# larskaislaniemi/PyLamp

Hardware: AMD Instinct MI355X
Metric: stokes_heat_mic_cell_updates_per_s (higher is better)
Workload: dtype f64

## Files before the change

pylamp_amd/csrc/pl_solver.hip:

```cpp
#include "pl_internal.h"
#include <chrono>
#include <cmath>
#include <functional>
#include <limits>

#define TB(tab, k) (tab)[(k) + PL_TOFF]

void pl_launch_heat_rhs(pl_ctx* ctx, const PlHeatOp& op, const double* Told, const double* H, double* rhs);

template <typename T>
struct PlVvOpT {
    PlGeom g;
    const T* etas; const T* etan;
    const T *rdz, *rDz, *rdx, *rDx;
    int slave_x;
    int slave_z0, slave_zL;
    T s0, sL;
    const T* szz; const T* szx;
};
typedef PlVvOpT<double> PlVvOp;
typedef PlVvOpT<float> PlVvOpF;

enum { VV_ZERO = 0, VV_INT = 1, VV_SLAVE = 2 };

// ... 1295 lines not shown
    float *etas_f = nullptr, *etan_f = nullptr, *tab_f = nullptr;
    float* vf[3] = {nullptr, nullptr, nullptr};
    float *ff = nullptr, *rf = nullptr;
};
template <typename T> struct LevelT;
template <> struct LevelT<double> {
    static const PlVvOp& op(const MgLevel* L) { return L->op; }
    static double** v(MgLevel* L) { return L->v; }
    static double* f(MgLevel* L) { return L->f; }
    static double* r(MgLevel* L) { return L->r; }
};
template <> struct LevelT<float> {
    static const PlVvOpF& op(const MgLevel* L) { return L->opf; }
    static float** v(MgLevel* L) { return L->vf; }
    static float* f(MgLevel* L) { return L->ff; }
    static float* r(MgLevel* L) { return L->rf; }
};

struct PlSolver {
    std::vector<MgLevel*> levels;
    int bc_key[4] = {-1, -1, -1, -1};
    int repl_start = -1;
    long long repl_max_nodes = 300000;
    double *r = nullptr, *rt = nullptr, *p = nullptr, *v = nullptr, *s = nullptr, *t = nullptr, *y = nullptr,
           *z = nullptr, *b = nullptr, *x = nullptr, *xb = nullptr, *dx = nullptr, *r0 = nullptr, *xh = nullptr,
           *bu = nullptr;
    double* scal = nullptr;
    double* hpart = nullptr;
    double* epi = nullptr;
    long long epi_blocks = 0;
    int nu_pre = 2, nu_post = 2, coarse_sweeps = 12;
    int nu0_pre = -1, nu0_post = -1;
    bool aniso_auto = true, ratio_knob = false;
    int power_its_warm = 1;
    bool nu_auto = true;
    bool use_tail = true;
    bool any_line = false;
    long long tail_knob = 0;
    long long tail_max_nodes = 33 * 33;
    int min_cells = 4;
    bool f32_enable = false; long long f32_min_nodes = 200000;
    double etol = 3e-8;
    double kappa = 1.0, sigma = 1.0;
    bool defl_enable = true;
    bool defl_persistent = false;
    bool defl_valid = false, defl_active = false;
    double *wdefl = nullptr, *udefl = nullptr;
    double defl_yAw = 0.0, defl_wvel2 = 0.0;
    double* Awdefl = nullptr;
    bool defl_lazy = false;
    double schur_scale = 1.0;
    double ref_cached = 0.0, ref_kc = 0.0; int ref_age = 0;
    long long fused_max_nodes = 1100000;
    long long tile32_min_nodes = 1000000;
    bool fused = true;
    bool fuse_first = true;
    bool l0_mixed = true;
    bool l0_mixed_now = true;
    bool deep = true;
    int tail_nu_pre = -1, tail_nu_post = -1;
    double cheb_ratio = 6.0, lmax_safety = 1.1;
    double* h[11] = {nullptr};
    double* hc3 = nullptr;
    double* hc[9] = {nullptr}; double* hc_part = nullptr; int hc_nb = 0, hc_last_its = 0;
    int napply = 0, nprec = 0;
    long long heat_fused_launches = 0;
    long long tail_lds_launches = 0, tail_global_launches = 0;
};

static PlSolver* solver_of(pl_ctx* ctx) {
    if (!ctx->krylov) {
        PlSolver* S = new PlSolver();
        if (const char* e = getenv("PYLAMP_MG_NU")) { int a = 0, b = 0; if (sscanf(e, "%d,%d", &a, &b) == 2 && a >= 0 && b >= 0 && a + b > 0) { S->nu_pre = a; S->nu_post = b; S->nu_auto = false; } }
        if (const char* e = getenv("PYLAMP_MG_NU0")) { int a = 0, b = 0; if (sscanf(e, "%d,%d", &a, &b) == 2 && a >= 1 && b >= 1) { S->nu0_pre = a; S->nu0_post = b; S->nu_auto = false; } }
        if (const char* e = getenv("PYLAMP_MG_POWER")) { int a = atoi(e); if (a >= 1) S->power_its_warm = a; }
        if (const char* e = getenv("PYLAMP_MG_COARSE")) { int a = atoi(e); if (a > 0) S->coarse_sweeps = a; }
        if (const char* e = getenv("PYLAMP_MG_TAIL")) S->use_tail = atoi(e) != 0;
        if (const char* e = getenv("PYLAMP_MG_REPL_NODES")) { long long v = atoll(e); if (v >= 25) S->repl_max_nodes = v; }
        if (const char* e = getenv("PYLAMP_MG_TAIL_NODES")) { long long v = atoll(e); if (v >= 25 && v <= PL_TAIL_MAX_NODES) S->tail_knob = v; }
        if (const char* e = getenv("PYLAMP_MG_DEEP")) S->deep = atoi(e) != 0;
        if (const char* e = getenv("PYLAMP_DEFLATE")) S->defl_enable = atoi(e) != 0;
        if (const char* e = getenv("PYLAMP_STOKES_ETOL")) { const double v = atof(e); if (v >= 0.0) S->etol = v; }
        if (const char* e = getenv("PYLAMP_MG_FP32")) S->f32_enable = atoi(e) != 0;
        if (const char* e = getenv("PYLAMP_MG_FP32_NODES")) { long long v = atoll(e); if (v >= 1) S->f32_min_nodes = v; }
        if (const char* e = getenv("PYLAMP_L0_MIXED")) S->l0_mixed = atoi(e) != 0;
        if (const char* e = getenv("PYLAMP_MG_FUSED")) S->fused = atoi(e) != 0;
        if (const char* e = getenv("PYLAMP_MG_TS32")) { long long v = atoll(e); if (v > 0) S->tile32_min_nodes = v; }
        if (const char* e = getenv("PYLAMP_MG_FUSED_MAX")) { long long v = atoll(e); if (v > 0) S->fused_max_nodes = v; }
        if (const char* e = getenv("PYLAMP_SCHUR_SCALE")) { double v = atof(e); if (v > 0.0) S->schur_scale = v; }
        if (const char* e = getenv("PYLAMP_MG_TAIL_NU")) { int a = 0, b = 0; if (sscanf(e, "%d,%d", &a, &b) == 2 && a + b > 0) { S->tail_nu_pre = a; S->tail_nu_post = b; } }
        if (const char* e = getenv("PYLAMP_MG_RATIO")) { double v = atof(e); if (v > 1.5) { S->cheb_ratio = v; S->ratio_knob = true; } }
        if (const char* e = getenv("PYLAMP_MG_ANISO")) S->aniso_auto = atoi(e) != 0;
        if (const char* e = getenv("PYLAMP_MG_SAFETY")) { double v = atof(e); if (v >= 1.0) S->lmax_safety = v; }
        ctx->krylov = S;
    }
    return (PlSolver*)ctx->krylov;
}

static void free_levels(PlSolver* S) {
    for (MgLevel* L : S->levels) {
        if (L->own_visc) { (void)hipFree(L->etas); (void)hipFree(L->etan); }
        if (L->own_rho && L->rho) (void)hipFree(L->rho);
        for (double* q : {L->szz, L->szx, L->eig}) if (q) (void)hipFree(q);
        for (double* q : {L->v[0], L->v[1], L->v[2], L->f, L->r}) if (q) (void)hipFree(q);
        for (float* q : {L->etas_f, L->etan_f, L->tab_f, L->vf[0], L->vf[1], L->vf[2], L->ff, L->rf}) if (q) (void)hipFree(q);
        pl_geom_free(L->gh);
        delete L;
// ... 656 lines not shown
            hipLaunchKernelGGL(k_vv_residual<T>, pl_grid_rows(V.op.g), dim3(64, 4), 0, ctx->stream, V.op, (const T*)(buf[0] - V.sh), f - V.sh,
                               r - V.sh, pl_row_iters(V.op.g));
    } else {
        smooth<T>(ctx, L, buf, f, npre, S->cheb_ratio, nullptr, 1.0, true, false, -1, first_done_anchor);
        if (L->dist) (void)pl_halo(ctx, g, buf[0], 2, g.plane);
        if (g_vv_vec)
            hipLaunchKernelGGL((k_vv_sweep2<1, T, T>), pl_grid_rows2(g), dim3(64, 4), 0, ctx->stream, LevelT<T>::op(L), (const T*)buf[0], (const T*)nullptr, f,
                               r, T(0), T(0), T(1));
        else
            hipLaunchKernelGGL(k_vv_residual<T>, pl_grid_rows(g), dim3(64, 4), 0, ctx->stream, LevelT<T>::op(L), (const T*)buf[0], f, r, pl_row_iters(g));
        if (L->dist) (void)pl_halo(ctx, g, r, 2, g.plane, 2);
    }
    if constexpr (std::is_same<T, float>::value) {
        if (C->f32) coarse_correction<float, float>(ctx, S, l, L, C, buf, deep, npost);
        else coarse_correction<float, double>(ctx, S, l, L, C, buf, deep, npost);
    } else {
        coarse_correction<double, double>(ctx, S, l, L, C, buf, deep, npost);
    }
    std::swap(buf[0], buf[2]);
    if (deep) *wrote_final = smooth<T>(ctx, L, buf, f, npost, S->cheb_ratio, final_out, final_scale, false, true, npost - 1);
    else *wrote_final = smooth<T>(ctx, L, buf, f, npost, S->cheb_ratio, final_out, final_scale, false, L->dist);
    *out = buf[0];
}

#define MGT_TS 16
#ifndef MGT_NT
#define MGT_NT 1024
#endif
struct MgTileArgs {
    PlVvOp op;
    PlVvOp opc;
    const double* f; double* fout;
    double* v;
    double* fc;
    const double* ec;
    double* out; double oscale; long long out_plane;
    double c1[4], c2[4];
    PlStokesOp sop; const double* rs; double* z;
    int tiles_x;
};

struct MgtTab { const double* es; const double* en; const double* rdz; const double* rDz; const double* rdx; const double* rDx; };

__device__ inline int mgt_cls_z(const PlVvOp& op, int i, int j, int& db, double& s) {
    db = 0; s = 1.0;
    if (i <= 0 || i >= op.g.nz - 1 || j < 0 || j >= op.g.nx - 1) return VV_ZERO;
    if (op.slave_x) {
        if (j == 0) { db = 1; return VV_SLAVE; }
        if (j == op.g.nx - 2) { db = -1; return VV_SLAVE; }
    }
    return VV_INT;
}
__device__ inline int mgt_cls_x(const PlVvOp& op, int i, int j, int& da, double& s) {
    da = 0; s = 1.0;
    if (j <= 0 || j >= op.g.nx - 1 || i < 0 || i >= op.g.nz - 1) return VV_ZERO;
    if (i == 0 && op.slave_z0) { da = 1; s = op.s0; return VV_SLAVE; }
    if (i == op.g.nz - 2 && op.slave_zL) { da = -1; s = op.sL; return VV_SLAVE; }
    return VV_INT;
}
__device__ inline void mgt_load_table(double* dst, const double* tab, int first_global, int count, int n) {
    for (int k = threadIdx.x; k < count; k += blockDim.x) {
        const int gk = first_global + k;
        dst[k] = (gk >= -PL_TOFF && gk < n + PL_TOFF) ? TB(tab, gk) : 0.0;
    }
}

struct MgtC { double c0, c1, c2, c3, x0, x1, rdg, s, f; int cm, d; bool on, interior; };
template <bool ZC>
__device__ inline MgtC mgt_classify(const PlVvOp& op, int CR, int NR, int ci0, int cj0, int a, int b) {
    MgtC k; k.c0 = k.c1 = k.c2 = k.c3 = k.x0 = k.x1 = k.rdg = k.f = 0.0; k.s = 1.0; k.cm = a * CR + b; k.d = 0; k.on = false; k.interior = false;
    if (a < 1 || a > NR - 2 || b < 1 || b > CR - 2) return k;
    int d; double s;
    const int cls = ZC ? mgt_cls_z(op, ci0 + a, cj0 + b, d, s) : mgt_cls_x(op, ci0 + a, cj0 + b, d, s);
    const int am = ZC ? a : a + d, bm = ZC ? b + d : b;
    if (cls == VV_ZERO || am < 1 || am > NR - 2 || bm < 1 || bm > CR - 2) return k;
    k.s = s; k.cm = am * CR + bm; k.d = d; k.on = true; k.interior = cls == VV_INT;
    return k;
}
template <bool ZC>
__device__ inline void mgt_coefficients(MgtC& k, const MgtTab& t, int CR) {
    if (!k.on) return;
    const int c = k.cm, am = c / CR, bm = c - am * CR;
    if (ZC) {
        const double rdz_i = t.rdz[am + 1], rdz_m = t.rdz[am], rDz_i = t.rDz[am + 1];
        const double rdx_j = t.rdx[bm + 1], rDx_j = t.rDx[bm + 1], rDx_p = t.rDx[bm + 2];
        const double esC = t.es[c], esE = t.es[c + 1];
        k.c0 = 4.0 * t.en[c] * rdz_i * rDz_i; k.c1 = 4.0 * t.en[c - CR] * rdz_m * rDz_i;
        k.c2 = 2.0 * esE * rDx_p * rdx_j; k.c3 = 2.0 * esC * rDx_j * rdx_j;
        k.x0 = 2.0 * esE * rDz_i * rdx_j; k.x1 = 2.0 * esC * rDz_i * rdx_j;
    } else {
        const double rdx_j = t.rdx[bm + 1], rdx_m = t.rdx[bm], rDx_j = t.rDx[bm + 1];
        const double rdz_i = t.rdz[am + 1], rDz_i = t.rDz[am + 1], rDz_p = t.rDz[am + 2];
        const double esC = t.es[c], esN = t.es[c + CR];
        k.c0 = 4.0 * t.en[c] * rdx_j * rDx_j; k.c1 = 4.0 * t.en[c - 1] * rdx_m * rDx_j;
        k.c2 = 2.0 * esN * rDz_p * rdz_i; k.c3 = 2.0 * esC * rDz_i * rdz_i;
        k.x0 = 2.0 * esN * rDx_j * rdz_i; k.x1 = 2.0 * esC * rDx_j * rdz_i;
    }
    k.rdg = pl_rcp(k.c0 + k.c1 + k.c2 + k.c3);
}
__device__ inline double mgt_dg(const MgtC& k) { return k.c0 + k.c1 + k.c2 + k.c3; }
__device__ inline double mgt_av_z(const MgtC& k, int CR, const double* vz, const double* vx, double& v0) {
    const int c = k.cm; v0 = vz[c];
    return k.c0 * (vz[c + CR] - v0) - k.c1 * (v0 - vz[c - CR]) + k.c2 * (vz[c + 1] - v0) - k.c3 * (v0 - vz[c - 1]) +
           k.x0 * (vx[c + 1] - vx[c - CR + 1]) - k.x1 * (vx[c] - vx[c - CR]);
}
__device__ inline double mgt_av_x(const MgtC& k, int CR, const double* vz, const double* vx, double& v0) {
    const int c = k.cm; v0 = vx[c];
    return k.c0 * (vx[c + 1] - v0) - k.c1 * (v0 - vx[c - 1]) + k.c2 * (vx[c + CR] - v0) - k.c3 * (v0 - vx[c - CR]) +
           k.x0 * (vz[c + CR] - vz[c + CR - 1]) - k.x1 * (vz[c] - vz[c - 1]);
}
__device__ inline void mgt_cheb(const MgtC& kz, const MgtC& kx, int CR, const double* vz, const double* vx, double& pvz, double& pvx,
                                double c1, double c2, double& oz, double& ox) {
    oz = 0.0; ox = 0.0;
    if (kz.on) {
        double v0; const double Av = mgt_av_z(kz, CR, vz, vx, v0);
        const double mom = (c1 != 0.0) ? c1 * (v0 - pvz) : 0.0;
        oz = kz.s * (v0 + mom + (c2 * (Av - kz.f)) * kz.rdg);
        pvz = v0;
    }
    if (kx.on) {
        double v0; const double Av = mgt_av_x(kx, CR, vz, vx, v0);
        const double mom = (c1 != 0.0) ? c1 * (v0 - pvx) : 0.0;
        ox = kx.s * (v0 + mom + (c2 * (Av - kx.f)) * kx.rdg);
        pvx = v0;
    }
}
__device__ inline bool mgt_owns(int ra, int rb, int HC, int TS, int i, int j, const PlGeom& g) {
    return ra >= HC && (ra < HC + TS || (ra == HC + TS && i == g.nz - 1)) && rb >= HC && (rb < HC + TS || (rb == HC + TS && j == g.nx - 1));
}
__host__ __device__ constexpr int mgt_npt(int nn) { return (nn + 1023) / 1024; }
__host__ __device__ constexpr int mgt_nt(int nn) { return ((nn + mgt_npt(nn) - 1) / mgt_npt(nn) + 63) / 64 * 64; }
__host__ __device__ constexpr int mgt_pre_nn(int NS, int TS) { return (TS + 2 * (NS + 2)) * (TS + 2 * (NS + 2)); }
__host__ __device__ constexpr int mgt_post_nn(int NS, int TS) { return (TS + 2 * (NS + 1)) * (TS + 2 * (NS + 1)); }

template <int NS, bool L0, int TS, int EXT = 0>
__global__ __launch_bounds__(mgt_nt(mgt_pre_nn(NS + EXT, TS))) void k_mg_pre(MgTileArgs a) {
    constexpr int H = NS + 1 + EXT, HC = H + 1, CR = TS + 2 * HC, NN = CR * CR, NPT = mgt_npt(NN), NT = mgt_nt(NN);
    __shared__ double V[2][2][NN];
    __shared__ double ZP[L0 ? NN : 1];
    __shared__ double TAB[4][CR + 4];
    double* const ES = V[1][0]; double* const EN = V[1][1];
    const PlGeom& g = a.op.g;
    const int tid = threadIdx.x;
    const int ty = blockIdx.x / a.tiles_x, tx = blockIdx.x % a.tiles_x;
    const int ti0 = g.gi0 + ty * TS, tj0 = g.gj0 + tx * TS;
    const int ci0 = ti0 - HC, cj0 = tj0 - HC;
    MgtTab t; t.es = ES; t.en = EN; t.rdz = TAB[0]; t.rDz = TAB[1]; t.rdx = TAB[2]; t.rDx = TAB[3];
    mgt_load_table(TAB[0], a.op.rdz, ci0 - 1, CR + 3, g.nz); mgt_load_table(TAB[1], a.op.rDz, ci0 - 1, CR + 3, g.nz);
    mgt_load_table(TAB[2], a.op.rdx, cj0 - 1, CR + 3, g.nx); mgt_load_table(TAB[3], a.op.rDx, cj0 - 1, CR + 3, g.nx);
    const long long P = g.plane;
    MgtC kz[NPT], kx[NPT];
    int depth[NPT];
#pragma unroll
    for (int q = 0; q < NPT; q++) {
        const int idx = tid + q * NT;
        const bool have = idx < NN;
        const int ra = have ? idx / CR : 0, rb = have ? idx % CR : 0, i = ci0 + ra, j = cj0 + rb;
        depth[q] = have ? min(min(ra, CR - 1 - ra), min(rb, CR - 1 - rb)) : -1;
        kz[q] = mgt_classify<true>(a.op, CR, CR, ci0, cj0, ra, rb);
        kx[q] = mgt_classify<false>(a.op, CR, CR, ci0, cj0, ra, rb);
        const bool inmem = i - g.gi0 >= -PL_RING && i - g.gi0 < g.lnz + PL_RING && j - g.gj0 >= -PL_RING && j - g.gj0 < g.lnx + PL_RING;
        const long long c = pl_idx(g, i - g.gi0, j - g.gj0);
        const double* const fsrc = L0 ? a.rs : a.f;
        if (kz[q].on) kz[q].f = fsrc[c + kz[q].d];
        if (kx[q].on) kx[q].f = fsrc[c + (long long)kx[q].d * g.pitch + P];
        if (have) {
            ES[idx] = inmem ? a.op.etas[c] : 0.0; EN[idx] = inmem ? a.op.etan[c] : 0.0;
            if (L0) {
                const bool indom = i >= 0 && i < g.nz && j >= 0 && j < g.nx;
                ZP[idx] = indom ? prec_p_value(a.sop, a.rs + 2 * P, i, j, c) : 0.0;
            }
        }
    }
    __syncthreads();
#pragma unroll
    for (int q = 0; q < NPT; q++) {
        mgt_coefficients<true>(kz[q], t, CR); mgt_coefficients<false>(kx[q], t, CR);
        if (L0) {
            const int idx = tid + q * NT;
            const int ra = depth[q] >= 0 ? idx / CR : 0, rb = depth[q] >= 0 ? idx % CR : 0, i = ci0 + ra, j = cj0 + rb;
            if (kz[q].on) kz[q].f = kz[q].f * mgt_dg(kz[q]) + 2.0 * a.sop.Kc * TAB[1][ra + 1] * (ZP[kz[q].cm] - ZP[kz[q].cm - CR]);
            if (kx[q].on) kx[q].f = kx[q].f * mgt_dg(kx[q]) + 2.0 * a.sop.Kc * TAB[3][rb + 1] * (ZP[kx[q].cm] - ZP[kx[q].cm - 1]);
            if (depth[q] >= 0 && mgt_owns(ra, rb, HC, TS, i, j, g) && i < g.nz && j < g.nx && i - g.gi0 < g.lnz && j - g.gj0 < g.lnx) {
                const long long c = pl_idx(g, i - g.gi0, j - g.gj0);
                a.fout[c] = kz[q].interior ? kz[q].f : 0.0; a.fout[c + P] = kx[q].interior ? kx[q].f : 0.0; a.z[c + 2 * P] = ZP[idx];
            }
        }
    }
    int cur = 0;
#pragma unroll
    for (int q = 0; q < NPT; q++) {
        const int idx = tid + q * NT;
        if (depth[q] >= HC - H) {
            V[0][0][idx] = kz[q].on ? (-kz[q].s * a.c2[0] * kz[q].f) * kz[q].rdg : 0.0;
            V[0][1][idx] = kx[q].on ? (-kx[q].s * a.c2[0] * kx[q].f) * kx[q].rdg : 0.0;
        }
    }
    __syncthreads();
    double pvz[NPT], pvx[NPT];
#pragma unroll
    for (int q = 0; q < NPT; q++) { pvz[q] = 0.0; pvx[q] = 0.0; }
#pragma unroll
    for (int k = 1; k < NS; k++) {
        const int h = H - k;
#pragma unroll
        for (int q = 0; q < NPT; q++) {
            const int idx = tid + q * NT;
            if (depth[q] >= HC - h) {
                double oz, ox;
                mgt_cheb(kz[q], kx[q], CR, V[cur][0], V[cur][1], pvz[q], pvx[q], a.c1[k], a.c2[k], oz, ox);
                V[cur ^ 1][0][idx] = oz; V[cur ^ 1][1][idx] = ox;
            }
        }
        __syncthreads();
        cur ^= 1;
    }
    const int nxt = cur ^ 1;
#pragma unroll
    for (int q = 0; q < NPT; q++) {
        const int idx = tid + q * NT;
        if (depth[q] >= HC - 1) {
            double v0, rz = 0.0, rx = 0.0;
            if (kz[q].interior) rz = kz[q].f - mgt_av_z(kz[q], CR, V[cur][0], V[cur][1], v0);
            if (kx[q].interior) rx = kx[q].f - mgt_av_x(kx[q], CR, V[cur][0], V[cur][1], v0);
            V[nxt][0][idx] = rz; V[nxt][1][idx] = rx;
        }
        if (depth[q] >= HC - (EXT ? NS : 1)) {
            const int ra = idx / CR, rb = idx % CR, i = ci0 + ra, j = cj0 + rb, li = i - g.gi0, lj = j - g.gj0;
            const bool owned = li >= 0 && li < g.lnz && lj >= 0 && lj < g.lnx;
            const bool ring = EXT && !owned && li >= -NS && li < g.lnz + NS && lj >= -NS && lj < g.lnx + NS;
            if (i >= 0 && i < g.nz && j >= 0 && j < g.nx && ((owned && mgt_owns(ra, rb, HC, TS, i, j, g)) || ring)) {
                const long long c = pl_idx(g, li, lj);
                a.v[c] = V[cur][0][idx]; a.v[c + P] = V[cur][1][idx];
            }
        }
    }
    __syncthreads();
    const PlGeom& gc = a.opc.g;
    for (int idx = tid; idx < (TS / 2 + 1) * (TS / 2 + 1); idx += NT) {
        const int u_ = idx / (TS / 2 + 1), w_ = idx % (TS / 2 + 1);
        const int I = (ti0 >> 1) + u_, J = (tj0 >> 1) + w_;
        if ((u_ == TS / 2 && I != gc.nz - 1) || (w_ == TS / 2 && J != gc.nx - 1)) continue;
        if (I >= gc.nz || J >= gc.nx || 2 * I - g.gi0 >= g.lnz || 2 * J - g.gj0 >= g.lnx) continue;
        const int b0 = (2 * I - ci0) * CR + (2 * J - cj0);
        int d; double s;
        double oz = 0.0, ox = 0.0;
        if (vv_cls_z(a.opc, I, J, d, s) == VV_INT) {
            const double wz[3] = {0.25, 0.5, 0.25}, wx[4] = {0.125, 0.375, 0.375, 0.125};
#pragma unroll
            for (int u = 0; u < 3; u++)
#pragma unroll
                for (int w = 0; w < 4; w++) oz += wz[u] * wx[w] * V[nxt][0][b0 + (u - 1) * CR + (w - 1)];
        }
        if (vv_cls_x(a.opc, I, J, d, s) == VV_INT) {
            const double wz[4] = {0.125, 0.375, 0.375, 0.125}, wx[3] = {0.25, 0.5, 0.25};
#pragma unroll
            for (int u = 0; u < 4; u++)
#pragma unroll
                for (int w = 0; w < 3; w++) ox += wz[u] * wx[w] * V[nxt][1][b0 + (u - 1) * CR + (w - 1)];
        }
        const long long cc = pl_idx(gc, I - gc.gi0, J - gc.gj0);
        a.fc[cc] = oz; a.fc[cc + gc.plane] = ox;
    }
}

template <int NS, int TS>
__global__ __launch_bounds__(mgt_nt(mgt_post_nn(NS, TS))) void k_mg_post(MgTileArgs a) {
    constexpr int H = NS, HC = H + 1, CR = TS + 2 * HC, NN = CR * CR, ECR = TS / 2 + H + 6, ENN = ECR * ECR, NPT = mgt_npt(NN), NT = mgt_nt(NN);
    __shared__ double V[2][2][NN];
    __shared__ double EC[2][ENN];
    __shared__ double TAB[4][CR + 4];
    double* const ES = V[0][0]; double* const EN = V[0][1];
    const PlGeom& g = a.op.g; const PlGeom& gc = a.opc.g;
    const int tid = threadIdx.x;
    const int ty = blockIdx.x / a.tiles_x, tx = blockIdx.x % a.tiles_x;
    const int ti0 = g.gi0 + ty * TS, tj0 = g.gj0 + tx * TS;
    const int ci0 = ti0 - HC, cj0 = tj0 - HC;
    MgtTab t; t.es = ES; t.en = EN; t.rdz = TAB[0]; t.rDz = TAB[1]; t.rdx = TAB[2]; t.rDx = TAB[3];
    mgt_load_table(TAB[0], a.op.rdz, ci0 - 1, CR + 3, g.nz); mgt_load_table(TAB[1], a.op.rDz, ci0 - 1, CR + 3, g.nz);
    mgt_load_table(TAB[2], a.op.rdx, cj0 - 1, CR + 3, g.nx); mgt_load_table(TAB[3], a.op.rDx, cj0 - 1, CR + 3, g.nx);
    const long long P = g.plane;
    const int eI0 = ((ti0 - H) >> 1) - 2, eJ0 = ((tj0 - H) >> 1) - 2;
    MgtC kz[NPT], kx[NPT];
    int depth[NPT];
#pragma unroll
    for (int q = 0; q < NPT; q++) {
        const int idx = tid + q * NT;
        const bool have = idx < NN;
        const int ra = have ? idx / CR : 0, rb = have ? idx % CR : 0, i = ci0 + ra, j = cj0 + rb;
        depth[q] = have ? min(min(ra, CR - 1 - ra), min(rb, CR - 1 - rb)) : -1;
        kz[q] = mgt_classify<true>(a.op, CR, CR, ci0, cj0, ra, rb);
        kx[q] = mgt_classify<false>(a.op, CR, CR, ci0, cj0, ra, rb);
        const bool inmem = i - g.gi0 >= -PL_RING && i - g.gi0 < g.lnz + PL_RING && j - g.gj0 >= -PL_RING && j - g.gj0 < g.lnx + PL_RING;
        const long long c = pl_idx(g, i - g.gi0, j - g.gj0);
        if (kz[q].on) kz[q].f = a.f[c + kz[q].d];
        if (kx[q].on) kx[q].f = a.f[c + (long long)kx[q].d * g.pitch + P];
        if (have) {
            ES[idx] = inmem ? a.op.etas[c] : 0.0; EN[idx] = inmem ? a.op.etan[c] : 0.0;
            V[1][0][idx] = inmem ? a.v[c] : 0.0; V[1][1][idx] = inmem ? a.v[c + P] : 0.0;
        }
    }
    for (int idx = tid; idx < ENN; idx += NT) {
        const int I = eI0 + idx / ECR, J = eJ0 + idx % ECR;
        const bool inmem = I - gc.gi0 >= -PL_RING && I - gc.gi0 < gc.lnz + PL_RING && J - gc.gj0 >= -PL_RING && J - gc.gj0 < gc.lnx + PL_RING;
        const long long cc = pl_idx(gc, I - gc.gi0, J - gc.gj0);
        EC[0][idx] = inmem ? a.ec[cc] : 0.0; EC[1][idx] = inmem ? a.ec[cc + gc.plane] : 0.0;
    }
    __syncthreads();
#pragma unroll
    for (int q = 0; q < NPT; q++) { mgt_coefficients<true>(kz[q], t, CR); mgt_coefficients<false>(kx[q], t, CR); }
    __syncthreads();
    auto ecz = [&](int I, int J) { return EC[0][(I - eI0) * ECR + (J - eJ0)]; };
    auto ecx = [&](int I, int J) { return EC[1][(I - eI0) * ECR + (J - eJ0)]; };
#pragma unroll
    for (int q = 0; q < NPT; q++) {
        const int idx = tid + q * NT;
        if (depth[q] >= HC - H) {
            const int ra = idx / CR, rb = idx % CR, i = ci0 + ra, j = cj0 + rb;
            int d; double s;
            double oz = 0.0, ox = 0.0;
            if (mgt_cls_z(a.op, i, j, d, s) != VV_ZERO) {
                const int jm = j + d;
                const int I0 = i >> 1, I1 = (i + 1) >> 1;
                int Jn = jm >> 1, Jo = (jm & 1) ? Jn + 1 : Jn - 1;
                Jn = min(max(Jn, 0), gc.nx - 2); Jo = min(max(Jo, 0), gc.nx - 2);
                const double pa = 0.5 * (ecz(I0, Jn) + ecz(I1, Jn)), pb = 0.5 * (ecz(I0, Jo) + ecz(I1, Jo));
                oz = s * (V[1][0][idx + d] + (0.75 * pa + 0.25 * pb));
            }
            if (mgt_cls_x(a.op, i, j, d, s) != VV_ZERO) {
                const int im = i + d;
                const int J0 = j >> 1, J1 = (j + 1) >> 1;
                int In = im >> 1, Io = (im & 1) ? In + 1 : In - 1;
                In = min(max(In, 0), gc.nz - 2); Io = min(max(Io, 0), gc.nz - 2);
                const double pa = 0.5 * (ecx(In, J0) + ecx(In, J1)), pb = 0.5 * (ecx(Io, J0) + ecx(Io, J1));
                ox = s * (V[1][1][idx + d * CR] + (0.75 * pa + 0.25 * pb));
            }
            V[0][0][idx] = oz; V[0][1][idx] = ox;
        }
    }
    __syncthreads();
    int cur = 0;
    double pvz[NPT], pvx[NPT];
#pragma unroll
    for (int q = 0; q < NPT; q++) { pvz[q] = 0.0; pvx[q] = 0.0; }
#pragma unroll
    for (int k = 0; k < NS; k++) {
        const int h = H - 1 - k;
#pragma unroll
        for (int q = 0; q < NPT; q++) {
            const int idx = tid + q * NT;
            if (depth[q] >= HC - h) {
                double oz, ox;
                mgt_cheb(kz[q], kx[q], CR, V[cur][0], V[cur][1], pvz[q], pvx[q], k == 0 ? 0.0 : a.c1[k], a.c2[k], oz, ox);
                if (k == NS - 1) {
                    const int ra = idx / CR, rb = idx % CR, i = ci0 + ra, j = cj0 + rb;
                    if (i < g.nz && j < g.nx && i - g.gi0 < g.lnz && j - g.gj0 < g.lnx) {
                        const long long c = pl_idx(g, i - g.gi0, j - g.gj0); a.out[c] = oz * a.oscale; a.out[c + a.out_plane] = ox * a.oscale;
                    }
                } else { V[cur ^ 1][0][idx] = oz; V[cur ^ 1][1][idx] = ox; }
            }
        }
        if (k < NS - 1) { __syncthreads(); cur ^= 1; }
    }
#pragma unroll
    for (int q = 0; q < NPT; q++) {
        const int idx = tid + q * NT;
        if (depth[q] == HC - 1) {
            const int ra = idx / CR, rb = idx % CR, i = ci0 + ra, j = cj0 + rb;
            if (mgt_owns(ra, rb, HC, TS, i, j, g) && i - g.gi0 < g.lnz && j - g.gj0 < g.lnx) {
                const long long c = pl_idx(g, i - g.gi0, j - g.gj0); a.out[c] = 0.0; a.out[c + a.out_plane] = 0.0;
            }
        }
    }
}

#define MGT_TAIL_POOL 18600
#define MGT_TAIL_CHEB 256
#define MGT_TAIL_LDS 11520
struct TailLvl { int base, NR, CR, N; };
#define TL_V(D, buf, c) (pool + (D).base + (2 * (buf) + (c)) * (D).N)
#define TL_ES(D) (pool + (D).base + 4 * (D).N)
#define TL_EN(D) (pool + (D).base + 5 * (D).N)
#define TL_TAB(D, k) (pool + (D).base + 6 * (D).N + ((k) < 2 ? (k) * ((D).NR + 3) : 2 * ((D).NR + 3) + ((k) - 2) * ((D).CR + 3)))
__host__ __device__ inline TailLvl mgt_tail_lvl(const PlGeom& g, int base) {
    TailLvl D; D.base = base; D.NR = g.nz + 2; D.CR = g.nx + 2; D.N = D.NR * D.CR;
    return D;
}
__host__ __device__ inline int mgt_tail_lvl_size(const TailLvl& D) { return 6 * D.N + 2 * (D.NR + 3) + 2 * (D.CR + 3); }
// ... 262 lines not shown
        need += 10LL * (g.nz + 2) * (g.nx + 2) + 2LL * (g.nz + 5) + 2LL * (g.nx + 5);
        lds += mgt_tail_lvl_size(mgt_tail_lvl(g, 0)); table_entries += 2LL * (g.nz + 5) + 2LL * (g.nx + 5);
        if (q > l) { coarse_threads = (coarse_threads + 63) / 64 * 64 + (long long)(g.nz - 1) * (g.nx - 1); coarse_nodes += (long long)g.nz * g.nx; }
    }
    const PlGeom& g0 = S->levels[l]->gh.d;
    return need <= MGT_TAIL_POOL && lds <= MGT_TAIL_LDS && (long long)(g0.nz - 1) * (g0.nx - 1) <= MGT_NT && (long long)g0.nz * g0.nx <= 2 * MGT_NT &&
           coarse_threads <= MGT_NT && coarse_nodes <= MGT_NT && table_entries <= MGT_NT;
}

static void cheb_coeffs(double lmax, double ratio, int n, double* c1, double* c2) {
    const double lmin = lmax / ratio, theta = 0.5 * (lmax + lmin), delta = 0.5 * (lmax - lmin), sigma = theta / delta;
    double rho_old = 1.0 / sigma;
    for (int k = 0; k < n; k++) {
        if (k == 0) { c1[k] = 0.0; c2[k] = 1.0 / theta; }
        else { const double rho = 1.0 / (2.0 * sigma - rho_old); c1[k] = rho * rho_old; c2[k] = 2.0 * rho / delta; rho_old = rho; }
    }
}
static bool mg_fused_level_ok(pl_ctx* ctx, const PlSolver* S, size_t l) {
    if (!S->fused || l + 1 >= S->levels.size() || S->any_line) return false;
    const MgLevel* L = S->levels[l];
    if (L->f32 || L->op.szz) return false;
    const PlGeom& g = L->gh.d;
    int npre_, npost_;
    level_nu(S, l, npre_, npost_);
    if (L->dist) {
        const bool dist_fused = !(getenv("PYLAMP_MG_FUSED_DIST") && atoi(getenv("PYLAMP_MG_FUSED_DIST")) == 0);
        const MgLevel* C = S->levels[l + 1];
        if (!dist_fused || l == 0 || npre_ + 2 > std::min(g.lnz, g.lnx) || npre_ + 3 > PL_RING) return false;
        if (C->dist && std::min(C->gh.d.lnz, C->gh.d.lnx) < 4) return false;
        if ((g.gi0 & 1) || (g.gj0 & 1)) return false;
    } else if (S->levels[l + 1]->dist) return false;
    if ((long long)g.lnz * g.lnx > S->fused_max_nodes) return false;
    if (S->use_tail && l > 0 && (long long)g.nz * g.nx <= S->tail_max_nodes && S->levels.size() - l <= PL_TAIL_MAX_LEVELS) return false;
    int npre, npost;
    level_nu(S, l, npre, npost);
    return npre >= 1 && npre <= 3 && npost >= 1 && npost <= 3;
}
static void vcycle_fused_level(pl_ctx* ctx, PlSolver* S, size_t l, const double* f, double** out, double* final_out, double final_scale,
                               const PlStokesOp* sop, const double* rs, double* z) {
    MgLevel* L = S->levels[l];
    MgLevel* C = S->levels[l + 1];
    const PlGeom& g = L->gh.d;
    int npre, npost;
    level_nu(S, l, npre, npost);
    MgTileArgs a{};
    a.op = L->op; a.opc = C->op;
    a.f = rs ? (const double*)L->f : f; a.fout = L->f; a.v = L->v[0]; a.fc = C->f;
    const int TS = (long long)g.lnz * g.lnx >= S->tile32_min_nodes ? 32 : MGT_TS;
    const int own_z = g.lnz - (g.gi0 + g.lnz == g.nz ? 1 : 0), own_x = g.lnx - (g.gj0 + g.lnx == g.nx ? 1 : 0);
    a.tiles_x = (own_x + TS - 1) / TS;
    const dim3 grid((unsigned)(a.tiles_x * ((own_z + TS - 1) / TS)));
    cheb_coeffs(L->lmax, S->cheb_ratio, npre, a.c1, a.c2);
    if (rs) { a.sop = *sop; a.rs = rs; a.z = z; }
#define MGT_PRE(NS, L0) do { if (TS == 32) hipLaunchKernelGGL((k_mg_pre<NS, L0, 32>), grid, dim3(mgt_nt(mgt_pre_nn(NS, 32))), 0, ctx->stream, a); \
                             else hipLaunchKernelGGL((k_mg_pre<NS, L0, MGT_TS>), grid, dim3(mgt_nt(mgt_pre_nn(NS, MGT_TS))), 0, ctx->stream, a); } while (0)
#define MGT_PRE_X(NS) do { if (TS == 32) hipLaunchKernelGGL((k_mg_pre<NS, false, 32, 1>), grid, dim3(mgt_nt(mgt_pre_nn(NS + 1, 32))), 0, ctx->stream, a); \
                           else hipLaunchKernelGGL((k_mg_pre<NS, false, MGT_TS, 1>), grid, dim3(mgt_nt(mgt_pre_nn(NS + 1, MGT_TS))), 0, ctx->stream, a); } while (0)
    if (L->dist) {
        (void)pl_halo(ctx, g, (double*)a.f, 2, g.plane, npre + 2);
        if (npre == 1) MGT_PRE_X(1); else if (npre == 2) MGT_PRE_X(2); else MGT_PRE_X(3);
        if (!C->dist) (void)pl_gather_blocks(ctx, C->gh.d, C->f, 2, C->gh.d.plane);
    }
    else if (rs) { if (npre == 1) MGT_PRE(1, true); else if (npre == 2) MGT_PRE(2, true); else MGT_PRE(3, true); }
    else { if (npre == 1) MGT_PRE(1, false); else if (npre == 2) MGT_PRE(2, false); else MGT_PRE(3, false); }
#undef MGT_PRE
#undef MGT_PRE_X
    double* ec = nullptr;
    bool wf = false;
    vcycle<double>(ctx, S, l + 1, C->f, &ec, &wf, nullptr, 1.0, 0, nullptr);
    if (L->dist && C->dist) (void)pl_halo(ctx, C->gh.d, ec, 2, C->gh.d.plane, 4);
    a.ec = ec; a.out = final_out ? final_out : L->v[2]; a.oscale = final_out ? final_scale : 1.0; a.out_plane = g.plane;
    cheb_coeffs(L->lmax, S->cheb_ratio, npost, a.c1, a.c2);
#define MGT_POST(NS) do { if (TS == 32) hipLaunchKernelGGL((k_mg_post<NS, 32>), grid, dim3(mgt_nt(mgt_post_nn(NS, 32))), 0, ctx->stream, a); \
                          else hipLaunchKernelGGL((k_mg_post<NS, MGT_TS>), grid, dim3(mgt_nt(mgt_post_nn(NS, MGT_TS))), 0, ctx->stream, a); } while (0)
    if (npost == 1) MGT_POST(1); else if (npost == 2) MGT_POST(2); else MGT_POST(3);
#undef MGT_POST
    *out = final_out ? nullptr : L->v[2];
}

template <typename T>
__global__ __launch_bounds__(256) void k_copy_vel(PlGeom g, const T* __restrict__ e, double* __restrict__ z, double oscale) {
    PL_NODE_PROLOGUE(g)
    (void)i; (void)j;
    z[c] = (double)e[c] * oscale; z[c + g.plane] = (double)e[c + g.plane] * oscale;
}

__global__ __launch_bounds__(256) void k_vv_close_frame(PlVvOp op, double* __restrict__ z) {
    const PlGeom& g = op.g;
    const int t = blockIdx.x * 256 + threadIdx.x;
    int i, j;
    if (t < 3 * g.lnx) { const int q = t / g.lnx; i = q == 0 ? 0 : g.nz - 3 + q; j = g.gj0 + t % g.lnx; }
    else if (t < 3 * g.lnx + 3 * g.lnz) { const int u = t - 3 * g.lnx, q = u / g.lnz; j = q == 0 ? 0 : g.nx - 3 + q; i = g.gi0 + u % g.lnz; }
    else return;
    const int li = i - g.gi0, lj = j - g.gj0;
    if (li < 0 || li >= g.lnz || lj < 0 || lj >= g.lnx) return;
    const long long c = pl_idx(g, li, lj), P = g.plane;
    int moff; double s;
    int cls = vv_cls_z(op, i, j, moff, s);
    if (cls == VV_ZERO) z[c] = 0.0; else if (cls == VV_SLAVE) z[c] = s * z[c + moff];
    cls = vv_cls_x(op, i, j, moff, s);
    if (cls == VV_ZERO) z[c + P] = 0.0; else if (cls == VV_SLAVE) z[c + P] = s * z[c + moff + P];
}

template <typename T>
static int stokes_precond_t(pl_ctx* ctx, PlSolver* S, const double* rs, double* z) {
    PlStokesOp op = ctx->sop;
    MgLevel* L0 = S->levels[0];
    MgLevel* L = L0;
    const PlGeom& g = ctx->sop.g;
    const bool f32 = std::is_same<T, float>::value;
    const double kappa = f32 ? S->kappa : 1.0, fscale = f32 ? S->kappa / S->sigma : 1.0, oscale = f32 ? 1.0 / S->kappa : 1.0;
    int e_last = 0, f_depth = 0;
    const bool deep = level_deep_plan(S, L0, 0, e_last, f_depth);
    ExtViewT<T> V = ext_view<T>(ctx, L0, deep ? f_depth : 0);
    if (L0->dist) {
        if (deep) PL_TRY(pl_halo(ctx, g, (double*)rs, 3, g.plane, f_depth + 1));
        else PL_TRY(pl_halo(ctx, g, (double*)rs + 2 * g.plane, 1, g.plane));
    }
    op.g = V.op.g; op.etas -= V.sh; op.etan -= V.sh; if (op.rho) op.rho -= V.sh;
// ... 1481 lines not shown
```

Measured before the change: 199.4 million.

## Batch all global loads into registers before shared-memory stores in multigrid tile kernels

Restructures the prologue of the fused multigrid pre/post smoothing kernels so every global load (viscosities, coordinate tables, RHS, velocities, coarse correction) is issued up front into registers, and only then written to shared memory. The goal is more memory-level parallelism and less serialized load latency per block. Table loads now use one wave per table, with wave-uniform branching and clamped addresses replacing predicated loads. It also lowers the node threshold for switching to 32-wide tiles, which costs more registers per thread and may reduce occupancy.

```diff
diff --git a/pylamp_amd/csrc/pl_solver.hip b/pylamp_amd/csrc/pl_solver.hip
--- a/pylamp_amd/csrc/pl_solver.hip
+++ b/pylamp_amd/csrc/pl_solver.hip
@@ -1371,7 +1371,7 @@
     double schur_scale = 1.0;
     double ref_cached = 0.0, ref_kc = 0.0; int ref_age = 0;
     long long fused_max_nodes = 1100000;
-    long long tile32_min_nodes = 1000000;
+    long long tile32_min_nodes = 250000;
     bool fused = true;
     bool fuse_first = true;
     bool l0_mixed = true;
@@ -2134,19 +2134,14 @@
     return VV_INT;
 }
 __device__ inline int mgt_cls_x(const PlVvOp& op, int i, int j, int& da, double& s) {
+    const double s0 = op.s0, sL = op.sL;
     da = 0; s = 1.0;
     if (j <= 0 || j >= op.g.nx - 1 || i < 0 || i >= op.g.nz - 1) return VV_ZERO;
-    if (i == 0 && op.slave_z0) { da = 1; s = op.s0; return VV_SLAVE; }
-    if (i == op.g.nz - 2 && op.slave_zL) { da = -1; s = op.sL; return VV_SLAVE; }
-    return VV_INT;
-}
-__device__ inline void mgt_load_table(double* dst, const double* tab, int first_global, int count, int n) {
-    for (int k = threadIdx.x; k < count; k += blockDim.x) {
-        const int gk = first_global + k;
-        dst[k] = (gk >= -PL_TOFF && gk < n + PL_TOFF) ? TB(tab, gk) : 0.0;
-    }
-}
-
+    if (i == 0 && op.slave_z0) da = 1;
+    else if (i == op.g.nz - 2 && op.slave_zL) da = -1;
+    s = da > 0 ? s0 : (da < 0 ? sL : 1.0);
+    return da ? VV_SLAVE : VV_INT;
+}
 struct MgtC { double c0, c1, c2, c3, x0, x1, rdg, s, f; int cm, d; bool on, interior; };
 template <bool ZC>
 __device__ inline MgtC mgt_classify(const PlVvOp& op, int CR, int NR, int ci0, int cj0, int a, int b) {
@@ -2215,6 +2210,99 @@
 __host__ __device__ constexpr int mgt_pre_nn(int NS, int TS) { return (TS + 2 * (NS + 2)) * (TS + 2 * (NS + 2)); }
 __host__ __device__ constexpr int mgt_post_nn(int NS, int TS) { return (TS + 2 * (NS + 1)) * (TS + 2 * (NS + 1)); }
 
+template <int NPT> struct MgtRawE { double es[NPT], en[NPT], tab; };
+template <int NPT> struct MgtRawF { double fz[NPT], fx[NPT]; };
+template <int NPT> struct MgtRawV { double vz[NPT], vx[NPT]; };
+struct MgtRawC { double ez, ex; };
+#define MGT_SLOT(q) const int idx = tid + (q) * NT; const bool have = idx < CR * CR; \
+    const int ra = have ? idx / CR : 0, rb = have ? idx % CR : 0, i = ci0 + ra, j = cj0 + rb; \
+    const bool inmem = have && i - g.gi0 >= -PL_RING && i - g.gi0 < g.lnz + PL_RING && j - g.gj0 >= -PL_RING && j - g.gj0 < g.lnx + PL_RING; \
+    const long long c = inmem ? pl_idx(g, i - g.gi0, j - g.gj0) : pl_idx(g, 0, 0);
+#define MGT_TAB_SLOT const int w = __builtin_amdgcn_readfirstlane(tid >> 6), k = tid & 63; \
+    const int gk = (w < 2 ? ci0 : cj0) - 1 + k, n = w < 2 ? g.nz : g.nx; \
+    const bool intab = w < 4 && k < CR + 3 && gk >= -PL_TOFF && gk < n + PL_TOFF;
+template <int NPT, int NT, int CR, int HC, int TS>
+__device__ inline void mgt_fetch_visc(MgtRawE<NPT>& r, const MgTileArgs& a, int tile, int tid) {
+    static_assert(CR + 3 <= 64 && NT >= 256, "one table per wave");
+    const PlGeom& g = a.op.g;
+    const int ci0 = g.gi0 + tile / a.tiles_x * TS - HC, cj0 = g.gj0 + tile % a.tiles_x * TS - HC;
+    MGT_TAB_SLOT
+    const double* const tab = w == 0 ? a.op.rdz : w == 1 ? a.op.rDz : w == 2 ? a.op.rdx : a.op.rDx;
+    r.tab = TB(tab, intab ? gk : -PL_TOFF);
+#pragma unroll
+    for (int q = 0; q < NPT; q++) {
+        MGT_SLOT(q)
+        r.es[q] = a.op.etas[c]; r.en[q] = a.op.etan[c];
+    }
+}
+template <int NPT, int NT, int CR, int HC, int TS>
+__device__ inline void mgt_store_visc(const MgtRawE<NPT>& r, const MgTileArgs& a, int tile, double* es, double* en, double* tab, int tid) {
+    const PlGeom& g = a.op.g;
+    const int ci0 = g.gi0 + tile / a.tiles_x * TS - HC, cj0 = g.gj0 + tile % a.tiles_x * TS - HC;
+#pragma unroll
+    for (int q = 0; q < NPT; q++) {
+        MGT_SLOT(q)
+        (void)c;
+        if (have) { es[idx] = inmem ? r.es[q] : 0.0; en[idx] = inmem ? r.en[q] : 0.0; }
+    }
+    MGT_TAB_SLOT
+    if (w < 4 && k < CR + 3) tab[w * (CR + 4) + k] = intab ? r.tab : 0.0;
+}
+template <int NPT, int NT, int CR, int HC, int TS>
+__device__ inline void mgt_fetch_rhs(MgtRawF<NPT>& r, const MgTileArgs& a, const double* fsrc, int tile, int tid) {
+    const PlGeom& g = a.op.g;
+    const int ci0 = g.gi0 + tile / a.tiles_x * TS - HC, cj0 = g.gj0 + tile % a.tiles_x * TS - HC;
+#pragma unroll
+    for (int q = 0; q < NPT; q++) {
+        MGT_SLOT(q)
+        const MgtC kz = mgt_classify<true>(a.op, CR, CR, ci0, cj0, ra, rb), kx = mgt_classify<false>(a.op, CR, CR, ci0, cj0, ra, rb);
+        const long long c0 = pl_idx(g, 0, 0), cn = pl_idx(g, i - g.gi0, j - g.gj0);
+        (void)c;
+        r.fz[q] = fsrc[kz.on ? cn + kz.d : c0];
+        r.fx[q] = fsrc[(kx.on ? cn + (long long)kx.d * g.pitch : c0) + g.plane];
+    }
+}
+template <int NPT, int NT, int CR, int HC, int TS>
+__device__ inline void mgt_fetch_v(MgtRawV<NPT>& r, const MgTileArgs& a, int tile, int tid) {
+    const PlGeom& g = a.op.g;
+    const int ci0 = g.gi0 + tile / a.tiles_x * TS - HC, cj0 = g.gj0 + tile % a.tiles_x * TS - HC;
+#pragma unroll
+    for (int q = 0; q < NPT; q++) {
+        MGT_SLOT(q)
+        r.vz[q] = a.v[c]; r.vx[q] = a.v[c + g.plane];
+    }
+}
+template <int NPT, int NT, int CR, int HC, int TS>
+__device__ inline void mgt_store_v(const MgtRawV<NPT>& r, const MgTileArgs& a, int tile, double* pvz, double* pvx, int tid) {
+    const PlGeom& g = a.op.g;
+    const int ci0 = g.gi0 + tile / a.tiles_x * TS - HC, cj0 = g.gj0 + tile % a.tiles_x * TS - HC;
+#pragma unroll
+    for (int q = 0; q < NPT; q++) {
+        MGT_SLOT(q)
+        (void)c;
+        if (have) { pvz[idx] = inmem ? r.vz[q] : 0.0; pvx[idx] = inmem ? r.vx[q] : 0.0; }
+    }
+}
+#define MGT_EC_SLOT const PlGeom& gc = a.opc.g; \
+    const int e = min(tid, ECR * ECR - 1), I = ((a.op.g.gi0 + tile / a.tiles_x * TS - H) >> 1) - 2 + e / ECR, J = ((a.op.g.gj0 + tile % a.tiles_x * TS - H) >> 1) - 2 + e % ECR; \
+    const bool inmem = I - gc.gi0 >= -PL_RING && I - gc.gi0 < gc.lnz + PL_RING && J - gc.gj0 >= -PL_RING && J - gc.gj0 < gc.lnx + PL_RING; \
+    const long long cc = inmem ? pl_idx(gc, I - gc.gi0, J - gc.gj0) : pl_idx(gc, 0, 0);
+template <int NT, int TS, int H, int ECR>
+__device__ inline void mgt_fetch_ec(MgtRawC& r, const MgTileArgs& a, int tile, int tid) {
+    static_assert(ECR * ECR <= NT, "one node of the coarse window per thread");
+    MGT_EC_SLOT
+    r.ez = a.ec[cc]; r.ex = a.ec[cc + gc.plane];
+}
+template <int NT, int TS, int H, int ECR>
+__device__ inline void mgt_store_ec(const MgtRawC& r, const MgTileArgs& a, int tile, double* ecz, double* ecx, int tid) {
+    MGT_EC_SLOT
+    (void)cc;
+    if (tid < ECR * ECR) { ecz[tid] = inmem ? r.ez : 0.0; ecx[tid] = inmem ? r.ex : 0.0; }
+}
+#undef MGT_EC_SLOT
+#undef MGT_SLOT
+#undef MGT_TAB_SLOT
+
 template <int NS, bool L0, int TS, int EXT = 0>
 __global__ __launch_bounds__(mgt_nt(mgt_pre_nn(NS + EXT, TS))) void k_mg_pre(MgTileArgs a) {
     constexpr int H = NS + 1 + EXT, HC = H + 1, CR = TS + 2 * HC, NN = CR * CR, NPT = mgt_npt(NN), NT = mgt_nt(NN);
@@ -2224,13 +2312,17 @@
     double* const ES = V[1][0]; double* const EN = V[1][1];
     const PlGeom& g = a.op.g;
     const int tid = threadIdx.x;
-    const int ty = blockIdx.x / a.tiles_x, tx = blockIdx.x % a.tiles_x;
+    MgtTab t; t.es = ES; t.en = EN; t.rdz = TAB[0]; t.rDz = TAB[1]; t.rdx = TAB[2]; t.rDx = TAB[3];
+    const long long P = g.plane;
+    const double* const fsrc = L0 ? a.rs : a.f;
+    MgtRawE<NPT> rawe;
+    MgtRawF<NPT> rawf;
+    mgt_fetch_visc<NPT, NT, CR, HC, TS>(rawe, a, blockIdx.x, tid);
+    mgt_fetch_rhs<NPT, NT, CR, HC, TS>(rawf, a, fsrc, blockIdx.x, tid);
+    mgt_store_visc<NPT, NT, CR, HC, TS>(rawe, a, blockIdx.x, ES, EN, TAB[0], tid);
+    const int tile = blockIdx.x, ty = tile / a.tiles_x, tx = tile % a.tiles_x;
     const int ti0 = g.gi0 + ty * TS, tj0 = g.gj0 + tx * TS;
     const int ci0 = ti0 - HC, cj0 = tj0 - HC;
-    MgtTab t; t.es = ES; t.en = EN; t.rdz = TAB[0]; t.rDz = TAB[1]; t.rdx = TAB[2]; t.rDx = TAB[3];
-    mgt_load_table(TAB[0], a.op.rdz, ci0 - 1, CR + 3, g.nz); mgt_load_table(TAB[1], a.op.rDz, ci0 - 1, CR + 3, g.nz);
-    mgt_load_table(TAB[2], a.op.rdx, cj0 - 1, CR + 3, g.nx); mgt_load_table(TAB[3], a.op.rDx, cj0 - 1, CR + 3, g.nx);
-    const long long P = g.plane;
     MgtC kz[NPT], kx[NPT];
     int depth[NPT];
 #pragma unroll
@@ -2241,17 +2333,12 @@
         depth[q] = have ? min(min(ra, CR - 1 - ra), min(rb, CR - 1 - rb)) : -1;
         kz[q] = mgt_classify<true>(a.op, CR, CR, ci0, cj0, ra, rb);
         kx[q] = mgt_classify<false>(a.op, CR, CR, ci0, cj0, ra, rb);
-        const bool inmem = i - g.gi0 >= -PL_RING && i - g.gi0 < g.lnz + PL_RING && j - g.gj0 >= -PL_RING && j - g.gj0 < g.lnx + PL_RING;
-        const long long c = pl_idx(g, i - g.gi0, j - g.gj0);
-        const double* const fsrc = L0 ? a.rs : a.f;
-        if (kz[q].on) kz[q].f = fsrc[c + kz[q].d];
-        if (kx[q].on) kx[q].f = fsrc[c + (long long)kx[q].d * g.pitch + P];
-        if (have) {
-            ES[idx] = inmem ? a.op.etas[c] : 0.0; EN[idx] = inmem ? a.op.etan[c] : 0.0;
-            if (L0) {
-                const bool indom = i >= 0 && i < g.nz && j >= 0 && j < g.nx;
-                ZP[idx] = indom ? prec_p_value(a.sop, a.rs + 2 * P, i, j, c) : 0.0;
-            }
+        if (kz[q].on) kz[q].f = rawf.fz[q];
+        if (kx[q].on) kx[q].f = rawf.fx[q];
+        if (L0 && have) {
+            const long long c = pl_idx(g, i - g.gi0, j - g.gj0);
+            const bool indom = i >= 0 && i < g.nz && j >= 0 && j < g.nx;
+            ZP[idx] = indom ? prec_p_value(a.sop, a.rs + 2 * P, i, j, c) : 0.0;
         }
     }
     __syncthreads();
@@ -2353,15 +2440,24 @@
     __shared__ double EC[2][ENN];
     __shared__ double TAB[4][CR + 4];
     double* const ES = V[0][0]; double* const EN = V[0][1];
+    double* const PVz = V[1][0]; double* const PVx = V[1][1];
     const PlGeom& g = a.op.g; const PlGeom& gc = a.opc.g;
     const int tid = threadIdx.x;
-    const int ty = blockIdx.x / a.tiles_x, tx = blockIdx.x % a.tiles_x;
+    MgtTab t; t.es = ES; t.en = EN; t.rdz = TAB[0]; t.rDz = TAB[1]; t.rdx = TAB[2]; t.rDx = TAB[3];
+    MgtRawV<NPT> rawv;
+    MgtRawC rawc;
+    MgtRawE<NPT> rawe;
+    MgtRawF<NPT> rawf;
+    mgt_fetch_v<NPT, NT, CR, HC, TS>(rawv, a, blockIdx.x, tid);
+    mgt_fetch_ec<NT, TS, H, ECR>(rawc, a, blockIdx.x, tid);
+    mgt_fetch_visc<NPT, NT, CR, HC, TS>(rawe, a, blockIdx.x, tid);
+    mgt_fetch_rhs<NPT, NT, CR, HC, TS>(rawf, a, a.f, blockIdx.x, tid);
+    mgt_store_v<NPT, NT, CR, HC, TS>(rawv, a, blockIdx.x, PVz, PVx, tid);
+    mgt_store_ec<NT, TS, H, ECR>(rawc, a, blockIdx.x, EC[0], EC[1], tid);
+    mgt_store_visc<NPT, NT, CR, HC, TS>(rawe, a, blockIdx.x, ES, EN, TAB[0], tid);
+    const int tile = blockIdx.x, ty = tile / a.tiles_x, tx = tile % a.tiles_x;
     const int ti0 = g.gi0 + ty * TS, tj0 = g.gj0 + tx * TS;
     const int ci0 = ti0 - HC, cj0 = tj0 - HC;
-    MgtTab t; t.es = ES; t.en = EN; t.rdz = TAB[0]; t.rDz = TAB[1]; t.rdx = TAB[2]; t.rDx = TAB[3];
-    mgt_load_table(TAB[0], a.op.rdz, ci0 - 1, CR + 3, g.nz); mgt_load_table(TAB[1], a.op.rDz, ci0 - 1, CR + 3, g.nz);
-    mgt_load_table(TAB[2], a.op.rdx, cj0 - 1, CR + 3, g.nx); mgt_load_table(TAB[3], a.op.rDx, cj0 - 1, CR + 3, g.nx);
-    const long long P = g.plane;
     const int eI0 = ((ti0 - H) >> 1) - 2, eJ0 = ((tj0 - H) >> 1) - 2;
     MgtC kz[NPT], kx[NPT];
     int depth[NPT];
@@ -2369,24 +2465,12 @@
     for (int q = 0; q < NPT; q++) {
         const int idx = tid + q * NT;
         const bool have = idx < NN;
-        const int ra = have ? idx / CR : 0, rb = have ? idx % CR : 0, i = ci0 + ra, j = cj0 + rb;
+        const int ra = have ? idx / CR : 0, rb = have ? idx % CR : 0;
         depth[q] = have ? min(min(ra, CR - 1 - ra), min(rb, CR - 1 - rb)) : -1;
         kz[q] = mgt_classify<true>(a.op, CR, CR, ci0, cj0, ra, rb);
         kx[q] = mgt_classify<false>(a.op, CR, CR, ci0, cj0, ra, rb);
-        const bool inmem = i - g.gi0 >= -PL_RING && i - g.gi0 < g.lnz + PL_RING && j - g.gj0 >= -PL_RING && j - g.gj0 < g.lnx + PL_RING;
-        const long long c = pl_idx(g, i - g.gi0, j - g.gj0);
-        if (kz[q].on) kz[q].f = a.f[c + kz[q].d];
-        if (kx[q].on) kx[q].f = a.f[c + (long long)kx[q].d * g.pitch + P];
-        if (have) {
-            ES[idx] = inmem ? a.op.etas[c] : 0.0; EN[idx] = inmem ? a.op.etan[c] : 0.0;
-            V[1][0][idx] = inmem ? a.v[c] : 0.0; V[1][1][idx] = inmem ? a.v[c + P] : 0.0;
-        }
-    }
-    for (int idx = tid; idx < ENN; idx += NT) {
-        const int I = eI0 + idx / ECR, J = eJ0 + idx % ECR;
-        const bool inmem = I - gc.gi0 >= -PL_RING && I - gc.gi0 < gc.lnz + PL_RING && J - gc.gj0 >= -PL_RING && J - gc.gj0 < gc.lnx + PL_RING;
-        const long long cc = pl_idx(gc, I - gc.gi0, J - gc.gj0);
-        EC[0][idx] = inmem ? a.ec[cc] : 0.0; EC[1][idx] = inmem ? a.ec[cc + gc.plane] : 0.0;
+        if (kz[q].on) kz[q].f = rawf.fz[q];
+        if (kx[q].on) kx[q].f = rawf.fx[q];
     }
     __syncthreads();
 #pragma unroll
@@ -2407,7 +2491,7 @@
                 int Jn = jm >> 1, Jo = (jm & 1) ? Jn + 1 : Jn - 1;
                 Jn = min(max(Jn, 0), gc.nx - 2); Jo = min(max(Jo, 0), gc.nx - 2);
                 const double pa = 0.5 * (ecz(I0, Jn) + ecz(I1, Jn)), pb = 0.5 * (ecz(I0, Jo) + ecz(I1, Jo));
-                oz = s * (V[1][0][idx + d] + (0.75 * pa + 0.25 * pb));
+                oz = s * (PVz[idx + d] + (0.75 * pa + 0.25 * pb));
             }
             if (mgt_cls_x(a.op, i, j, d, s) != VV_ZERO) {
                 const int im = i + d;
@@ -2415,7 +2499,7 @@
                 int In = im >> 1, Io = (im & 1) ? In + 1 : In - 1;
                 In = min(max(In, 0), gc.nz - 2); Io = min(max(Io, 0), gc.nz - 2);
                 const double pa = 0.5 * (ecx(In, J0) + ecx(In, J1)), pb = 0.5 * (ecx(Io, J0) + ecx(Io, J1));
-                ox = s * (V[1][1][idx + d * CR] + (0.75 * pa + 0.25 * pb));
+                ox = s * (PVx[idx + d * CR] + (0.75 * pa + 0.25 * pb));
             }
             V[0][0][idx] = oz; V[0][1][idx] = ox;
         }
@@ -2784,19 +2868,16 @@
     const dim3 grid((unsigned)(a.tiles_x * ((own_z + TS - 1) / TS)));
     cheb_coeffs(L->lmax, S->cheb_ratio, npre, a.c1, a.c2);
     if (rs) { a.sop = *sop; a.rs = rs; a.z = z; }
-#define MGT_PRE(NS, L0) do { if (TS == 32) hipLaunchKernelGGL((k_mg_pre<NS, L0, 32>), grid, dim3(mgt_nt(mgt_pre_nn(NS, 32))), 0, ctx->stream, a); \
-                             else hipLaunchKernelGGL((k_mg_pre<NS, L0, MGT_TS>), grid, dim3(mgt_nt(mgt_pre_nn(NS, MGT_TS))), 0, ctx->stream, a); } while (0)
-#define MGT_PRE_X(NS) do { if (TS == 32) hipLaunchKernelGGL((k_mg_pre<NS, false, 32, 1>), grid, dim3(mgt_nt(mgt_pre_nn(NS + 1, 32))), 0, ctx->stream, a); \
-                           else hipLaunchKernelGGL((k_mg_pre<NS, false, MGT_TS, 1>), grid, dim3(mgt_nt(mgt_pre_nn(NS + 1, MGT_TS))), 0, ctx->stream, a); } while (0)
+#define MGT_PRE(NS, L0, EXT) do { if (TS == 32) hipLaunchKernelGGL((k_mg_pre<NS, L0, 32, EXT>), grid, dim3(mgt_nt(mgt_pre_nn(NS + EXT, 32))), 0, ctx->stream, a); \
+                                  else hipLaunchKernelGGL((k_mg_pre<NS, L0, MGT_TS, EXT>), grid, dim3(mgt_nt(mgt_pre_nn(NS + EXT, MGT_TS))), 0, ctx->stream, a); } while (0)
     if (L->dist) {
         (void)pl_halo(ctx, g, (double*)a.f, 2, g.plane, npre + 2);
-        if (npre == 1) MGT_PRE_X(1); else if (npre == 2) MGT_PRE_X(2); else MGT_PRE_X(3);
+        if (npre == 1) MGT_PRE(1, false, 1); else if (npre == 2) MGT_PRE(2, false, 1); else MGT_PRE(3, false, 1);
         if (!C->dist) (void)pl_gather_blocks(ctx, C->gh.d, C->f, 2, C->gh.d.plane);
     }
-    else if (rs) { if (npre == 1) MGT_PRE(1, true); else if (npre == 2) MGT_PRE(2, true); else MGT_PRE(3, true); }
-    else { if (npre == 1) MGT_PRE(1, false); else if (npre == 2) MGT_PRE(2, false); else MGT_PRE(3, false); }
+    else if (rs) { if (npre == 1) MGT_PRE(1, true, 0); else if (npre == 2) MGT_PRE(2, true, 0); else MGT_PRE(3, true, 0); }
+    else { if (npre == 1) MGT_PRE(1, false, 0); else if (npre == 2) MGT_PRE(2, false, 0); else MGT_PRE(3, false, 0); }
 #undef MGT_PRE
-#undef MGT_PRE_X
     double* ec = nullptr;
     bool wf = false;
     vcycle<double>(ctx, S, l + 1, C->f, &ec, &wf, nullptr, 1.0, 0, nullptr);
```

Measured after the change: 203.7 million, median of 6. 2.2% higher.
